# kkty/kmer-sets-compression

Hardware: AMD Instinct MI355X
Metric: Mk-mers/s processed in kmerset-multiple-compress; bytes/k-mer after SPSS (higher is better)
Workload: dtype u32

## Files before the change

kmer-sets-compression_amd/csrc/ksh_encode.hip:

```cpp
#include "ksh_internal.h"
#include "ksh_dsu.h"
#include "ksh_kmer.h"

#include <algorithm>
#include <cstddef>
#include <cstdlib>
#include <string>

namespace ksh {

#ifndef KSH_RULER_SHIFT
#define KSH_RULER_SHIFT 5
#endif
constexpr int kRulerShift = KSH_RULER_SHIFT;
constexpr uint32_t kRulerEvery = 1u << kRulerShift;

constexpr uint32_t kNone = 0xFFFFFFFFu;
constexpr uint32_t kMulti = 0xFFFFFFFEu;

#ifndef KSH_JUMP_HOPS
#define KSH_JUMP_HOPS 4
#endif
constexpr int kJumpHops = KSH_JUMP_HOPS;

#ifdef KSH_TRACE
__device__ unsigned long long* g_probe_trace = nullptr;
__device__ long long g_probe_trace_rows = 0;
#define KSH_PMARK(which, m)                                                                              \
  do {                                                                                                   \
    if (g_probe_trace && threadIdx.x == 0 && int64_t(blockIdx.x) < g_probe_trace_rows)                    \
      g_probe_trace[((which) * g_probe_trace_rows + blockIdx.x) * 16 + (m)] = __builtin_amdgcn_s_memtime(); \
  } while (0)
#define KSH_PMARK_WAVE(which)                                                                            \
  do {                                                                                                   \
    if (g_probe_trace && threadIdx.x % 64 == 0 && threadIdx.x / 64 < 16 && int64_t(blockIdx.x) < g_probe_trace_rows) \
      g_probe_trace[((which) * g_probe_trace_rows + blockIdx.x) * 16 + threadIdx.x / 64] = __builtin_amdgcn_s_memtime(); \
  } while (0)
#else
#define KSH_PMARK(which, m) do { } while (0)
#define KSH_PMARK_WAVE(which) do { } while (0)
// ... 186 lines not shown
                                                      const uint32_t* __restrict__ hist_matrix,
                                                      const int64_t* __restrict__ goff,
                                                      RcRecord<KeyT>* __restrict__ rec) {
  extern __shared__ uint32_t lds_hist[];
  const int nb = 1 << nbits;
  const uint32_t* my_row = hist_matrix + int64_t(blockIdx.x) * nb;
  for (int b = threadIdx.x; b < nb; b += blockDim.x) lds_hist[b] = uint32_t(goff[b]) + my_row[b];
  const int64_t t_begin = int64_t(blockIdx.x) * per_row;
  const int64_t t_end = min(t_begin + per_row, set.n);
  __syncthreads();
  if (t_begin >= t_end) return;
  const int64_t b_first = set.bucket_of(t_begin), b_last = set.bucket_of(t_end - 1);
  const int k = set.k, low_bits = 2 * set.k - 2 - nbits;
  const uint64_t low_mask = (uint64_t(1) << low_bits) - 1;
  for (int64_t t = t_begin + threadIdx.x; t < t_end; t += blockDim.x) {
    const uint64_t key = uint64_t(set.keys[t]);
    const uint32_t grp = uint32_t(revcomp(key, k) >> low_bits) & uint32_t(nb - 1);
    if (int(grp >> (nbits - round_bits)) != round) continue;
    int64_t lo = b_first, hi = b_last;
    while (lo < hi) {
      const int64_t mid = (lo + hi + 1) >> 1;
      if (set.off[mid] <= t) lo = mid; else hi = mid - 1;
    }
    const uint64_t rx = revcomp((uint64_t(lo) << set.key_bits) | key, k);
    const uint32_t dst = atomicAdd(&lds_hist[grp], 1u);
    RcRecord<KeyT> r;
    r.key = KeyT(((rx >> (2 * k - 2)) << low_bits) | (rx & low_mask));
    r.t = uint32_t(t);
    rec[dst] = r;
  }
}

constexpr int kSgBits = 7;
constexpr int kL1Threads = 1024;
constexpr int kL2Threads = 256;
constexpr int kL2Per = 8;
constexpr int kL2Tile = kL2Threads * kL2Per;

template <typename KeyT, int kPer>
__global__ __launch_bounds__(kL1Threads) void k_rc_scatter_l1(DevSet<KeyT> set, int nbits, int64_t per_row,
                                                               const uint32_t* __restrict__ hist_matrix,
                                                               const int64_t* __restrict__ goff,
                                                               RcRecord<KeyT>* __restrict__ tmp_rec,
                                                               uint16_t* __restrict__ tmp_g) {
  constexpr int kTile = kL1Threads * kPer;
  constexpr int kSg = 1 << kSgBits;
  __shared__ RcRecord<KeyT> s_rec[kTile];
  __shared__ uint16_t s_g[kTile];
  __shared__ uint32_t s_cur[kSg], s_cnt[kSg], s_lbase[kSg + 1];
  constexpr int kOffCap = 1024;
  __shared__ int64_t s_off[kOffCap];
  const int tid = threadIdx.x;
  const int nb = 1 << nbits, lo_bits = nbits - kSgBits;
  const uint32_t* my_row = hist_matrix + int64_t(blockIdx.x) * nb;
  if (tid < kSg) {
    uint32_t at = uint32_t(goff[int64_t(tid) << lo_bits]);
    for (int gi = 0; gi < (1 << lo_bits); gi++) at += my_row[(tid << lo_bits) + gi];
    s_cur[tid] = at;
    s_cnt[tid] = 0;
  }
  const int64_t t_begin = int64_t(blockIdx.x) * per_row;
  const int64_t t_end = min(t_begin + per_row, set.n);
  __syncthreads();
  if (t_begin >= t_end) return;
  const int64_t b_first = set.bucket_of(t_begin), b_last = set.bucket_of(t_end - 1);
  const int k = set.k, low_bits = 2 * set.k - 2 - nbits;
  const uint64_t low_mask = (uint64_t(1) << low_bits) - 1;
  const int n_span = int(min<int64_t>(b_last - b_first + 1, kOffCap + 1));
  const bool off_staged = n_span <= kOffCap;
  if (off_staged)
    for (int j = tid; j < n_span; j += kL1Threads) s_off[j] = set.off[b_first + j];
  __syncthreads();
  for (int64_t t0 = t_begin; t0 < t_end; t0 += kTile) {
    const int tile_n = int(min<int64_t>(kTile, t_end - t0));
    RcRecord<KeyT> mine[kPer];
    uint32_t grp[kPer], rank[kPer];
#pragma unroll
    for (int j = 0; j < kPer; j++) {
      const int64_t t = t0 + tid + j * kL1Threads;
      grp[j] = 0xFFFFFFFFu;
      if (t >= t_end) continue;
      const uint64_t key = uint64_t(set.keys[t]);
      int64_t lo = b_first, hi = b_last;
      if (off_staged) {
        int l2 = 0, h2 = n_span - 1;
        while (l2 < h2) {
          const int mid = (l2 + h2 + 1) >> 1;
          if (s_off[mid] <= t) l2 = mid; else h2 = mid - 1;
        }
        lo = b_first + l2;
      } else {
        while (lo < hi) {
          const int64_t mid = (lo + hi + 1) >> 1;
          if (set.off[mid] <= t) lo = mid; else hi = mid - 1;
        }
      }
      const uint64_t rx = revcomp((uint64_t(lo) << set.key_bits) | key, k);
      grp[j] = uint32_t(rx >> low_bits) & uint32_t(nb - 1);
      mine[j].key = KeyT(((rx >> (2 * k - 2)) << low_bits) | (rx & low_mask));
      mine[j].t = uint32_t(t);
      rank[j] = atomicAdd(&s_cnt[grp[j] >> lo_bits], 1u);
    }
    __syncthreads();
    if (tid < 64) {
      static_assert(kSg == 128, "two super-groups per lane of one wave");
      const uint32_t c0 = s_cnt[2 * tid], c1 = s_cnt[2 * tid + 1];
      uint32_t inc = c0 + c1;
#pragma unroll
      for (int d = 1; d < 64; d <<= 1) {
        const uint32_t o = __shfl_up(inc, d, 64);
        if (tid >= d) inc += o;
      }
      s_lbase[2 * tid] = inc - c0 - c1;
      s_lbase[2 * tid + 1] = inc - c1;
    }
    __syncthreads();
#pragma unroll
    for (int j = 0; j < kPer; j++) {
      if (grp[j] == 0xFFFFFFFFu) continue;
      const uint32_t pos = s_lbase[grp[j] >> lo_bits] + rank[j];
      s_rec[pos] = mine[j];
      s_g[pos] = uint16_t(grp[j]);
    }
    __syncthreads();
    for (int i = tid; i < tile_n; i += kL1Threads) {
      const uint32_t sg = uint32_t(s_g[i]) >> lo_bits;
      const uint32_t dst = s_cur[sg] + (uint32_t(i) - s_lbase[sg]);
      tmp_rec[dst] = s_rec[i];
      tmp_g[dst] = s_g[i];
    }
    __syncthreads();
    if (tid < kSg) {
      s_cur[tid] += s_cnt[tid];
      s_cnt[tid] = 0;
    }
    __syncthreads();
  }
}

template <typename KeyT>
__global__ __launch_bounds__(kL2Threads) void k_rc_scatter_l2(int64_t n, int nbits, const int64_t* __restrict__ goff,
                                                               const RcRecord<KeyT>* __restrict__ tmp_rec,
                                                               const uint16_t* __restrict__ tmp_g,
                                                               uint32_t* __restrict__ cursor,
                                                               RcRecord<KeyT>* __restrict__ rec) {
  constexpr int kBins = 512;
  __shared__ RcRecord<KeyT> s_rec[kL2Tile];
  __shared__ uint16_t s_bin[kL2Tile];
  __shared__ uint32_t s_cnt[kBins], s_lbase[kBins], s_gbase[kBins];
  __shared__ uint32_t s_first;
  const int tid = threadIdx.x;
  const int lo_bits = nbits - kSgBits;
  const int64_t p0 = int64_t(blockIdx.x) * kL2Tile;
  const int tile_n = int(min<int64_t>(kL2Tile, n - p0));
  for (int b = tid; b < kBins; b += kL2Threads) s_cnt[b] = 0;
  if (tid == 0) s_first = (uint32_t(tmp_g[p0]) >> lo_bits) << lo_bits;
  __syncthreads();
  const uint32_t base_g = s_first;
  const uint32_t n_bins = min<uint32_t>(uint32_t(kBins), (2u << lo_bits));
  RcRecord<KeyT> mine[kL2Per];
  uint32_t bin[kL2Per], rank[kL2Per];
#pragma unroll
  for (int j = 0; j < kL2Per; j++) {
    const int i = tid + j * kL2Threads;
    bin[j] = 0xFFFFFFFFu;
    if (i >= tile_n) continue;
    mine[j] = tmp_rec[p0 + i];
    const uint32_t g = tmp_g[p0 + i];
    if (g - base_g < n_bins) {
      bin[j] = g - base_g;
      rank[j] = atomicAdd(&s_cnt[bin[j]], 1u);
    } else {
      rec[uint32_t(goff[g]) + atomicAdd(&cursor[g], 1u)] = mine[j];
    }
  }
  __syncthreads();
  {
    static_assert(kBins == 2 * kL2Threads, "two bins per thread");
    __shared__ uint32_t s_wave[kL2Threads / 64];
    const uint32_t c0 = s_cnt[2 * tid], c1 = s_cnt[2 * tid + 1];
    uint32_t inc = c0 + c1;
    const int lane = tid & 63, wv = tid >> 6;
#pragma unroll
    for (int d = 1; d < 64; d <<= 1) {
      const uint32_t o = __shfl_up(inc, d, 64);
      if (lane >= d) inc += o;
    }
    if (lane == 63) s_wave[wv] = inc;
    __syncthreads();
    uint32_t before = inc - (c0 + c1);
    for (int w = 0; w < wv; w++) before += s_wave[w];
    s_lbase[2 * tid] = before;
    s_lbase[2 * tid + 1] = before + c0;
    s_gbase[2 * tid] = c0 ? uint32_t(goff[base_g + 2 * tid]) + atomicAdd(&cursor[base_g + 2 * tid], c0) : 0u;
    s_gbase[2 * tid + 1] = c1 ? uint32_t(goff[base_g + 2 * tid + 1]) + atomicAdd(&cursor[base_g + 2 * tid + 1], c1) : 0u;
  }
  __syncthreads();
#pragma unroll
  for (int j = 0; j < kL2Per; j++) {
    if (bin[j] == 0xFFFFFFFFu) continue;
    const uint32_t pos = s_lbase[bin[j]] + rank[j];
// ... 1124 lines not shown
}

__device__ __forceinline__ unsigned long long rec_look(const unsigned long long* p) {
  return __hip_atomic_load(p, __ATOMIC_RELAXED, __HIP_MEMORY_SCOPE_AGENT);
}
__device__ __forceinline__ void rec_post(unsigned long long* p, unsigned long long v) {
  __hip_atomic_store(p, v, __ATOMIC_RELAXED, __HIP_MEMORY_SCOPE_AGENT);
}
__device__ __forceinline__ bool first_phase(uint32_t s) {
  return (((s >> 1) * 0x9E3779B1u) >> 13 ^ s) & 1u;
}

struct WalkLog {
  unsigned long long* hdr;
  uint32_t* mid;
  int64_t n_walkers;
  int n_mid;
  int k;
  uint32_t* long_walkers;
  unsigned int* long_count;
  uint32_t long_tag;
  __device__ __forceinline__ bool is_long(uint32_t steps) const { return steps > uint32_t(n_mid + 1) * uint32_t(k); }
  __device__ __forceinline__ void arrived(int64_t w, uint32_t steps, uint32_t state) const {
    if (!hdr) return;
    hdr[w] = (uint64_t(steps) << 32) | state;
    if (is_long(steps)) long_walkers[atomicAdd(long_count, 1u)] = uint32_t(w) | long_tag;
  }
  __device__ __forceinline__ void passed(int64_t w, int j, uint32_t state) const {
    if (hdr && j < n_mid) mid[int64_t(j) * n_walkers + w] = state;
  }
};
constexpr int kLogMidRulers = 7, kLogMidHeads = 7;

template <int kPhase>
__global__ __launch_bounds__(256) void k_rank_walk(const uint32_t* __restrict__ link, int64_t n_states,
                                                    int64_t n_dense, unsigned long long* __restrict__ rinfo,
                                                    unsigned long long* __restrict__ chain_info, WalkLog log,
                                                    unsigned long long* __restrict__ unset_a,
                                                    unsigned long long* __restrict__ unset_b) {
  const int64_t i = int64_t(blockIdx.x) * blockDim.x + threadIdx.x;
  if (i >= n_dense) return;
  if (unset_a) {
    unset_a[i] = ~0ull;
    unset_b[i] = ~0ull;
  }
  const int64_t s64 = 2 * int64_t(kRulerEvery) * (i >> 1) + (i & 1);
  if (s64 >= n_states) {
    rinfo[i] = make_rinfo(true, 0, 0);
    return;
  }
  const uint32_t r = uint32_t(s64);
  if (kPhase == 1 && !first_phase(r)) return;
  if (rec_look(rinfo + i) != kRecUnset) return;
  const uint2 own = link_pair(link, r);
  uint32_t lk = leave_link(own, r);
  if (lk == kNone) {
    rec_post(rinfo + i, make_rinfo(true, 0, r));
    if (enter_link(own, r) == kNone) log.arrived(i, 0, r);
    return;
  }
  uint32_t cur = r, steps = 0;
  int since = 0, n_passed = 0;
  while (true) {
    cur = step_to(cur, lk);
    steps++;
    if (sampled_ruler(cur) || steps >= 0x3FFFFFFFu) {
      rec_post(rinfo + i, make_rinfo(false, steps, cur));
      rec_post(rinfo + dense_index(cur ^ 1), make_rinfo(false, steps, r ^ 1));
      log.arrived(i, steps, cur);
      return;
    }
    if (++since == log.k) {
      since = 0;
      log.passed(i, n_passed++, cur);
    }
    lk = leave_link(link_pair(link, cur), cur);
    if (lk == kNone) {
      rec_post(rinfo + i, make_rinfo(true, steps, cur));
      rec_post(chain_info + (cur >> 1), make_chain_info(true, steps, dense_index(r ^ 1)));
      log.arrived(i, steps, cur);
      return;
    }
  }
}

template <int kPhase>
__global__ __launch_bounds__(256) void k_rank_heads(const uint32_t* __restrict__ link,
                                                     const uint32_t* __restrict__ ends, int64_t n_ends,
                                                     unsigned long long* __restrict__ rinfo,
                                                     unsigned long long* __restrict__ chain_info, WalkLog log) {
  const int64_t e = int64_t(blockIdx.x) * blockDim.x + threadIdx.x;
  if (e >= n_ends) return;
  const uint32_t t = ends[e];
  if ((t & (kRulerEvery - 1)) == 0) return;
  const uint2 own = reinterpret_cast<const uint2*>(link)[t];
  uint32_t s0;
  if (own.x == kNone && own.y != kNone) {
    s0 = 2 * t;
  } else if (own.y == kNone && own.x != kNone) {
    s0 = 2 * t + 1;
  } else {
    log.arrived(e, 0, 2 * t);
    return;
  }
  if (kPhase == 1 && !first_phase(s0)) return;
  if (rec_look(chain_info + t) != kRecUnset) return;
  uint32_t lk = leave_link(own, s0);
  uint32_t cur = s0, off = 0;
  int since = 0, n_passed = 0;
  while (true) {
    cur = step_to(cur, lk);
    off++;
    if (sampled_ruler(cur)) {
      rec_post(chain_info + t, make_chain_info(true, off, dense_index(cur)));
      rec_post(rinfo + dense_index(cur ^ 1), make_rinfo(true, off, s0 ^ 1));
      log.arrived(e, off, cur);
      return;
    }
    if (++since == log.k) {
      since = 0;
      log.passed(e, n_passed++, cur);
    }
    lk = leave_link(link_pair(link, cur), cur);
    if (lk == kNone || off >= 0x3FFFFFFFu) {
      rec_post(chain_info + t, make_chain_info(false, off, cur));
      rec_post(chain_info + (cur >> 1), make_chain_info(false, off, s0 ^ 1));
      log.arrived(e, off, cur);
      return;
    }
  }
}

__global__ __launch_bounds__(256) void k_rank_unset(const uint32_t* __restrict__ ends, int64_t n_ends,
                                                     unsigned long long* __restrict__ chain_info) {
  const int64_t e = int64_t(blockIdx.x) * blockDim.x + threadIdx.x;
  if (e < n_ends) chain_info[ends[e]] = kRecUnset;
}

__global__ __launch_bounds__(256) void k_ruler_jump(int64_t n_dense,
                                                     unsigned long long* __restrict__ rinfo,
                                                     const int* __restrict__ prev,
                                                     int* __restrict__ changed) {
  if (prev && *prev == 0) return;
  const int64_t i = int64_t(blockIdx.x) * blockDim.x + threadIdx.x;
  if (i >= n_dense) return;
  uint64_t mine = rinfo[i];
  if (mine & kEndFlag) return;
#pragma unroll
  for (int hop = 0; hop < kJumpHops && !(mine & kEndFlag); hop++) {
    const uint64_t theirs = rinfo[dense_index(uint32_t(mine))];
    const uint32_t dist = uint32_t((mine >> 32) & 0x7FFFFFFFu) + uint32_t((theirs >> 32) & 0x7FFFFFFFu);
    mine = (theirs & kEndFlag) | (uint64_t(dist & 0x7FFFFFFFu) << 32) | uint32_t(theirs);
  }
  rinfo[i] = mine;
  *changed = 1;
}

#ifndef KSH_L2_SHIFT
#define KSH_L2_SHIFT 4
#endif
constexpr int kL2Shift = KSH_L2_SHIFT;
// ... 1193 lines not shown
  uint32_t *u_head = nullptr, *u_first = nullptr, *u_last = nullptr, *u_len = nullptr,
           *edges = nullptr, *mate = nullptr, *best_w = nullptr, *u_sid = nullptr,
           *u_koff = nullptr, *lens = nullptr, *sc_nodes = nullptr, *sc_parent = nullptr,
           *sc_rank = nullptr;
  unsigned long long *best_prio = nullptr, *sc_used = nullptr;
  uint8_t *visited = nullptr, *scls = nullptr, *u_flip = nullptr;
  int64_t *s_nk = nullptr, *sc01 = nullptr, *sc2 = nullptr, *str_start = nullptr;
  EncCtl* ctl = nullptr;
  int rounds = 0;
  int64_t routes = 0;
  bool stamped = true;
  bool directed = false;
  const unsigned long long *rinfo = nullptr, *chain_info = nullptr;
  const uint32_t* ends = nullptr;
  int64_t n_ends = 0;
  WalkLog log_rulers{}, log_heads{};
  bool cover = false;
  ksh_spss_view in{};
  int64_t* in_start = nullptr;
  bool ready = false;
  bool written = false;
  bool ambiguous = false;
};

inline size_t al(size_t x) { return (x + 255) & ~size_t(255); }

#define KSH_BOUND(cond)                                                                              \
  do {                                                                                               \
    if (!(cond)) return ::ksh::fail(KSH_INTERNAL, "encode: bound violated: %s (%s:%d)", #cond, __FILE__, __LINE__); \
  } while (0)
static_assert(sizeof(RcRecord<uint16_t>) == 8 && sizeof(RcRecord<uint32_t>) == 8 && sizeof(RcRecord<uint64_t>) == 16,
              "record sizes the scratch layout assumes");

constexpr int64_t kRcRowsMax = 512;
constexpr int64_t kRcWindowBytes = 78 << 10;

inline bool staged_adjacency() {
  static const bool on = [] {
    const char* e = getenv("KSH_ADJACENCY");
    return !(e && std::string(e) == "probe");
  }();
  return on;
}
inline bool rank_with_stamps() {
  static const bool on = [] {
    const char* e = getenv("KSH_RANK");
    return e && std::string(e) == "stamp";
  }();
  return on;
}
inline bool emit_by_walking() {
  static const bool on = [] {
    const char* e = getenv("KSH_EMIT");
    return e && std::string(e) == "walk";
  }();
  return on;
}
inline int64_t l2_threshold() {
  static const int64_t v = [] {
    const char* e = getenv("KSH_L2_MIN");
    return e ? std::max<int64_t>(4096, atoll(e)) : int64_t(1) << 20;
  }();
  return v;
}
inline unsigned nblk(int64_t n) { return unsigned(std::max<int64_t>(1, (n + 255) / 256)); }

template <typename T>
T* carve(char*& at, size_t count) {
  T* p = reinterpret_cast<T*>(at);
  at += al(count * sizeof(T));
  return p;
}

void free_plan(ksh_ctx* ctx) {
  EncPlan* p = static_cast<EncPlan*>(ctx->enc_state);
  if (!p) return;
  if (p->ublock) pool_free(ctx, p->ublock);
  delete p;
  ctx->enc_state = nullptr;
}

static bool replaces_unwritten(const ksh_ctx* ctx, bool cover) {
  const EncPlan* o = static_cast<const EncPlan*>(ctx->enc_state);
  return o && o->ready && !o->written && o->cover == cover;
}

void retire_plan(ksh_ctx* ctx) {
  if (EncPlan* p = static_cast<EncPlan*>(ctx->enc_state)) p->ready = false;
}

static int enc_fine_bits(const ksh_geom* g, int64_t n) {
  const int64_t nb = n_buckets(g);
  int fine_bits = 0;
  while (fine_bits < 13 && fine_bits + 2 < key_bits(g) && (int64_t(3) << fine_bits) < 2 * (n / nb + 1)) fine_bits++;
  return fine_bits;
}
// ... 176 lines not shown
        const uint32_t bit = 1u << (sizeof(KeyT) == 2 ? 0 : sizeof(KeyT) == 4 ? 1 : 2);
        if (!(ctx->lds_opt_in & bit)) {
          const int bytes = int(kRcWindowBytes + 2048);
          KSH_HIP(hipFuncSetAttribute(reinterpret_cast<const void*>(k_adj_rc<KeyT, 1024>),
                                      hipFuncAttributeMaxDynamicSharedMemorySize, bytes));
          KSH_HIP(hipFuncSetAttribute(reinterpret_cast<const void*>(k_adj_rc<KeyT, 512>),
                                      hipFuncAttributeMaxDynamicSharedMemorySize, bytes));
          KSH_HIP(hipFuncSetAttribute(reinterpret_cast<const void*>(k_adj_rc<KeyT, 256>),
                                      hipFuncAttributeMaxDynamicSharedMemorySize, bytes));
          KSH_HIP(hipFuncSetAttribute(reinterpret_cast<const void*>(k_adj_rc<KeyT, 64>),
                                      hipFuncAttributeMaxDynamicSharedMemorySize, bytes));
          KSH_HIP(hipFuncSetAttribute(reinterpret_cast<const void*>(k_adj_rc1<KeyT, 1024>),
                                      hipFuncAttributeMaxDynamicSharedMemorySize, kRc1LdsBytes));
          KSH_HIP(hipFuncSetAttribute(reinterpret_cast<const void*>(k_adj_rc1<KeyT, 512>),
                                      hipFuncAttributeMaxDynamicSharedMemorySize, kRc1LdsBytes));
          KSH_HIP(hipFuncSetAttribute(reinterpret_cast<const void*>(k_adj_rc1<KeyT, 256>),
                                      hipFuncAttributeMaxDynamicSharedMemorySize, kRc1LdsBytes));
          KSH_HIP(hipFuncSetAttribute(reinterpret_cast<const void*>(k_adj_rc1<KeyT, 64>),
                                      hipFuncAttributeMaxDynamicSharedMemorySize, kRc1LdsBytes));
          KSH_HIP(hipFuncSetAttribute(reinterpret_cast<const void*>(k_rc_hist<KeyT>),
                                      hipFuncAttributeMaxDynamicSharedMemorySize, int(size_t(4) << 15)));
          ctx->lds_opt_in |= bit;
        }
      }
      KSH_BOUND(hist_lds <= (size_t(4) << 15) && ng <= 65536);
      hipLaunchKernelGGL((k_rc_hist<KeyT>), dim3(unsigned(rows)), dim3(1024), hist_lds, st,
                         static_cast<const KeyT*>(sv->d_keys), n, g->k, key_bits(g), gbits, per_row, hist);
      hipLaunchKernelGGL(k_rc_columns, dim3(unsigned((ng + 63) / 64)), dim3(64 * kColTeams), 0, st, hist, rows, int(ng),
                         totals);
      KSH_TRY(scan_exclusive_i64(ctx, totals, goff, ng, goff + ng));
      p->routes |= KSH_ROUTE_PROBE_STAGED | (two_level ? KSH_ROUTE_SCATTER_TWO_LEVEL : 0);
      if (two_level) {
        RcRecord<KeyT>* tmp_rec = sizeof(RcRecord<KeyT>) == 8 ? rec + n : reinterpret_cast<RcRecord<KeyT>*>(p->nbr);
        uint16_t* tmp_g = reinterpret_cast<uint16_t*>(p->head);
        KSH_BOUND(sizeof(RcRecord<KeyT>) == 8 ? size_t(2 * n) * sizeof(RcRecord<KeyT>) <= al(size_t(2 * n) * 8)
                                    : reinterpret_cast<char*>(p->link) == reinterpret_cast<char*>(p->nbr) + al(size_t(2 * n) * 4) &&
                                          size_t(n) * sizeof(RcRecord<KeyT>) <= 2 * al(size_t(2 * n) * 4));
        KSH_BOUND(gbits - kSgBits <= 8);
        uint32_t* cursor = rc_cursor;
        constexpr int kPer = sizeof(RcRecord<KeyT>) == 8 ? 4 : 2;
        hipLaunchKernelGGL((k_rc_scatter_l1<KeyT, kPer>), dim3(unsigned(rows)), dim3(kL1Threads), 0, st, set, gbits,
                           per_row, hist, goff, tmp_rec, tmp_g);
        hipLaunchKernelGGL((k_rc_scatter_l2<KeyT>), dim3(unsigned((n + kL2Tile - 1) / kL2Tile)), dim3(kL2Threads), 0,
                           st, n, gbits, goff, tmp_rec, tmp_g, cursor, rec);
      } else {
        hipLaunchKernelGGL((k_rc_scatter<KeyT>), dim3(unsigned(rows)), dim3(1024), hist_lds, st, set, gbits, 0, 0,
                           per_row, hist, goff, rec);
      }
      const int64_t per_group = n / ng;
      const int cap = int(std::min<int64_t>((kRcWindowBytes - 4 * kRcSegs) / int64_t(sizeof(KeyT) + 6),
                                            std::max<int64_t>(1024, extra ? per_group * 23 / 20 + 256 : per_group * 5 / 4 + 256))) & ~7;
      const size_t rc_lds = size_t(cap) * (sizeof(KeyT) + 4) + size_t(cap + 2 * kRcSegs) * 2;
      KSH_BOUND(cap >= 8 && cap % 8 == 0 && cap + 2 * kRcSegs < 65536);
      KSH_BOUND(rc_lds + 2048 <= size_t(kRcWindowBytes) + 2048 && rc_lds <= size_t(kRcWindowBytes));
      int64_t* pb = static_cast<int64_t*>(arena_alloc(ctx, size_t(ng) * 2 * kRcSegs * 8));
      int64_t* pb0 = extra ? static_cast<int64_t*>(arena_alloc(ctx, size_t(ng) * 2 * 8)) : nullptr;
      if (!pb || (extra && !pb0)) return fail(KSH_INTERNAL, "scratch arena too small");
      hipLaunchKernelGGL((k_rc_bounds<KeyT>), dim3(nblk(ng * 2 * kRcSegs + (extra ? ng * 2 : 0))), dim3(256), 0, st, set,
                         gbits, pb, pb0);
      p->routes |= per_group > 4096 ? KSH_ROUTE_RC_1024 : per_group > 1024 ? KSH_ROUTE_RC_512
                   : per_group > 256 ? KSH_ROUTE_RC_256 : KSH_ROUTE_RC_64;
      static const int rc1_mode = [] {
        const char* e = getenv("KSH_RC1");
        return !e ? 1 : (std::string(e) == "marks" ? 2 : (std::string(e) == "batched" ? 0 : 1));
      }();
      const bool rc1_marks = rc1_mode == 2;
      const int rc1_cap = rc1_marks ? 0 : int(std::min<int64_t>(Rc1Cfg<KeyT>::kCap, (per_group * 4 / 3 + 263) & ~int64_t(7)));
      const int pass1_cap = rc1_marks ? -1 : rc1_cap;
      const bool with_rc = rc1_mode != 0;
      int rc1_sbits = 6;
      while ((1 << rc1_sbits) < kRc1SlicesMax && (2 << rc1_sbits) <= rc1_cap + 1) rc1_sbits++;
      const size_t rc1_lds = (size_t(4) << rc1_sbits) + size_t(rc1_cap) * Rc1Cfg<KeyT>::kEntryBytes;
      KSH_BOUND(rc1_lds <= size_t(kRc1LdsBytes) && rc1_cap % 8 == 0 && rc1_cap < (2 << rc1_sbits) - 1);
      if (!rc1_marks) p->routes |= KSH_ROUTE_RC1_STREAMED;
      const int rc1_batched = rc1_mode == 0 ? 1 : 0;
#define KSH_LAUNCH_RC(T)                                                                                              \
  do {                                                                                                                \
// ... 101 lines not shown
        lr.k = lh.k = g->k;
        const size_t used = (size_t(n_dense) + size_t(n)) * 8;
        const size_t log_bytes = size_t(n_dense) * (8 + 4 * kLogMidRulers + 4) + size_t(n_ends) * (8 + 4 * kLogMidHeads + 4) + 64;
        if (!emit_by_walking() && used + log_bytes <= size_t(2 * n) * 8) {
          unsigned long long* at8 = p->info + n_dense + n;
          lr.hdr = at8;
          lh.hdr = at8 + n_dense;
          uint32_t* at4 = reinterpret_cast<uint32_t*>(at8 + n_dense + n_ends);
          lr.mid = at4;
          lh.mid = at4 + size_t(kLogMidRulers) * n_dense;
          lr.long_walkers = lh.long_walkers = lh.mid + size_t(kLogMidHeads) * n_ends;
          lr.long_count = lh.long_count = ctl->long_count;
          lr.long_tag = 0;
          lh.long_tag = kLongHead;
          lr.n_walkers = n_dense;
          lh.n_walkers = n_ends;
          lr.n_mid = kLogMidRulers;
          lh.n_mid = kLogMidHeads;
          KSH_HIP(hipMemsetAsync(at8, 0xFF, size_t(n_dense + n_ends) * 8, st));
          p->routes |= KSH_ROUTE_EMIT_LOGS;
        }
        p->log_rulers = lr;
        p->log_heads = lh;
        KSH_HIP(hipMemsetAsync(rinfo, 0xFF, size_t(n_dense) * 8, st));
        hipLaunchKernelGGL(k_rank_unset, dim3(nblk(n_ends)), dim3(256), 0, st, ends, n_ends, chain_info);
        static const int64_t race_min = [] {
          const char* e = getenv("KSH_RANK_PHASES");
          if (e && std::string(e) == "1") return int64_t(0);
          if (e && std::string(e) == "2") return int64_t(1) << 60;
          const char* m = getenv("KSH_RANK_RACE_MIN");
          return m ? int64_t(atoll(m)) : int64_t(1) << 18;
        }();
        p->routes |= (n_dense >= race_min ? KSH_ROUTE_RANK_ONE_LAUNCH : 0) | (n_ends >= race_min ? KSH_ROUTE_HEADS_ONE_LAUNCH : 0);
        if (n_dense < race_min)
          hipLaunchKernelGGL(k_rank_walk<1>, dim3(nblk(n_dense)), dim3(256), 0, st, link, ns2, n_dense, rinfo, chain_info, lr,
                             static_cast<unsigned long long*>(nullptr), static_cast<unsigned long long*>(nullptr));
        if (n_ends < race_min)
          hipLaunchKernelGGL(k_rank_heads<1>, dim3(nblk(n_ends)), dim3(256), 0, st, link, ends, n_ends, rinfo, chain_info, lh);
        const bool l2_after = n_dense >= l2_threshold();
        hipLaunchKernelGGL(k_rank_walk<2>, dim3(nblk(n_dense)), dim3(256), 0, st, link, ns2, n_dense, rinfo, chain_info, lr,
                           l2_after ? reinterpret_cast<unsigned long long*>(p->hlen) : nullptr,
                           l2_after ? reinterpret_cast<unsigned long long*>(p->hlast) : nullptr);
        hipLaunchKernelGGL(k_rank_heads<2>, dim3(nblk(n_ends)), dim3(256), 0, st, link, ends, n_ends, rinfo, chain_info, lh);
      }
    }
    const bool two_levels = !stamped && n_dense >= l2_threshold();
    const int64_t n_jump = two_levels ? (((n_dense - 1) >> (kL2Shift + 1)) << 1) + 2 : n_dense;
    unsigned long long* r2 = reinterpret_cast<unsigned long long*>(p->uid);
    unsigned long long* l2_head = reinterpret_cast<unsigned long long*>(p->hlen);
    unsigned long long* l2_stamp = reinterpret_cast<unsigned long long*>(p->hlast);
    if (two_levels) p->routes |= KSH_ROUTE_JUMP_TWO_LEVEL;
    if (stamped) p->routes = (p->routes | KSH_ROUTE_RANK_STAMPED) & ~int64_t(KSH_ROUTE_EMIT_LOGS | KSH_ROUTE_RANK_ONE_LAUNCH | KSH_ROUTE_HEADS_ONE_LAUNCH | KSH_ROUTE_JUMP_TWO_LEVEL);
    if (two_levels) {
      hipLaunchKernelGGL(k_l2_walk<true>, dim3(nblk(n_jump)), dim3(256), 0, st, rinfo, n_dense, r2, l2_head, l2_stamp);
      hipLaunchKernelGGL(k_l2_walk<false>, dim3(nblk(n_dense)), dim3(256), 0, st, rinfo, n_dense, r2, l2_head, l2_stamp);
    }
    int max_rounds = 3;
    for (int64_t x = n_jump; x > 1; x /= (kJumpHops + 1)) max_rounds++;
    max_rounds = std::min(max_rounds, kJumpRoundsMax);
    if (!first_pass) {
      KSH_HIP(hipMemsetAsync(ctl->jump_live, 0, sizeof(ctl->jump_live), st));
      KSH_HIP(hipMemsetAsync(d_tot, 0, (3 + kLenSums) * 8, st));
      KSH_HIP(hipMemsetAsync(ctl->long_count, 0, sizeof(ctl->long_count), st));
    }
    for (int round = 0; round < max_rounds; round++) {
      const int* prev = round ? &ctl->jump_live[round - 1] : nullptr;
      if (two_levels)
        hipLaunchKernelGGL(k_l2_jump, dim3(nblk(n_jump)), dim3(256), 0, st, n_jump, r2, prev, &ctl->jump_live[round]);
      else
        hipLaunchKernelGGL(k_ruler_jump, dim3(nblk(n_dense)), dim3(256), 0, st, n_dense, rinfo, prev,
                           &ctl->jump_live[round]);
    }
    if (two_levels)
      hipLaunchKernelGGL(k_l2_resolve, dim3(nblk(n_dense)), dim3(256), 0, st, n_dense, r2, l2_head, l2_stamp, rinfo);
    int* loop_flag = reinterpret_cast<int*>(d_tot + 2 + kLenSums);
    if (stamped) {
// ... 451 lines not shown
```

Before: 27820.

## Drop tmp_g side array by packing group low bits into record t field

The first scatter level stops writing a separate 16-bit group array. It packs the group's low bits together with a row-relative index into the record's t field and publishes per-row, per-supergroup start offsets. The second level recovers the supergroup and source row by binary searching goff and those shared starts, then rebuilds the global index and group. This removes one global write and one read stream per record, at the cost of extra binary-search work per element and new range constraints on per_row.

```diff
diff --git a/kmer-sets-compression_amd/csrc/ksh_encode.hip b/kmer-sets-compression_amd/csrc/ksh_encode.hip
--- a/kmer-sets-compression_amd/csrc/ksh_encode.hip
+++ b/kmer-sets-compression_amd/csrc/ksh_encode.hip
@@ -258,6 +258,7 @@
 }
 
 constexpr int kSgBits = 7;
+constexpr int64_t kRcRowsMax = 512;
 constexpr int kL1Threads = 1024;
 constexpr int kL2Threads = 256;
 constexpr int kL2Per = 8;
@@ -268,7 +269,7 @@
                                                                const uint32_t* __restrict__ hist_matrix,
                                                                const int64_t* __restrict__ goff,
                                                                RcRecord<KeyT>* __restrict__ tmp_rec,
-                                                               uint16_t* __restrict__ tmp_g) {
+                                                               uint32_t* __restrict__ share) {
   constexpr int kTile = kL1Threads * kPer;
   constexpr int kSg = 1 << kSgBits;
   __shared__ RcRecord<KeyT> s_rec[kTile];
@@ -284,6 +285,7 @@
     for (int gi = 0; gi < (1 << lo_bits); gi++) at += my_row[(tid << lo_bits) + gi];
     s_cur[tid] = at;
     s_cnt[tid] = 0;
+    share[int64_t(tid) * gridDim.x + blockIdx.x] = at;
   }
   const int64_t t_begin = int64_t(blockIdx.x) * per_row;
   const int64_t t_end = min(t_begin + per_row, set.n);
@@ -292,6 +294,7 @@
   const int64_t b_first = set.bucket_of(t_begin), b_last = set.bucket_of(t_end - 1);
   const int k = set.k, low_bits = 2 * set.k - 2 - nbits;
   const uint64_t low_mask = (uint64_t(1) << low_bits) - 1;
+  const uint32_t g_low_mask = (1u << lo_bits) - 1u;
   const int n_span = int(min<int64_t>(b_last - b_first + 1, kOffCap + 1));
   const bool off_staged = n_span <= kOffCap;
   if (off_staged)
@@ -324,7 +327,7 @@
       const uint64_t rx = revcomp((uint64_t(lo) << set.key_bits) | key, k);
       grp[j] = uint32_t(rx >> low_bits) & uint32_t(nb - 1);
       mine[j].key = KeyT(((rx >> (2 * k - 2)) << low_bits) | (rx & low_mask));
-      mine[j].t = uint32_t(t);
+      mine[j].t = (uint32_t(t - t_begin) << lo_bits) | (grp[j] & g_low_mask);
       rank[j] = atomicAdd(&s_cnt[grp[j] >> lo_bits], 1u);
     }
     __syncthreads();
@@ -353,7 +356,6 @@
       const uint32_t sg = uint32_t(s_g[i]) >> lo_bits;
       const uint32_t dst = s_cur[sg] + (uint32_t(i) - s_lbase[sg]);
       tmp_rec[dst] = s_rec[i];
-      tmp_g[dst] = s_g[i];
     }
     __syncthreads();
     if (tid < kSg) {
@@ -364,25 +366,55 @@
   }
 }
 
+template <typename T>
+__device__ __forceinline__ int last_at_most(const T* a, int lo, int hi, uint32_t p, int64_t stride = 1) {
+  while (lo < hi) {
+    const int mid = (lo + hi + 1) >> 1;
+    if (uint32_t(a[mid * stride]) <= p) lo = mid; else hi = mid - 1;
+  }
+  return lo;
+}
+
 template <typename KeyT>
-__global__ __launch_bounds__(kL2Threads) void k_rc_scatter_l2(int64_t n, int nbits, const int64_t* __restrict__ goff,
+__global__ __launch_bounds__(kL2Threads) void k_rc_scatter_l2(int64_t n, int nbits, int64_t per_row, int n_rows,
+                                                               const int64_t* __restrict__ goff,
                                                                const RcRecord<KeyT>* __restrict__ tmp_rec,
-                                                               const uint16_t* __restrict__ tmp_g,
+                                                               const uint32_t* __restrict__ share,
                                                                uint32_t* __restrict__ cursor,
                                                                RcRecord<KeyT>* __restrict__ rec) {
   constexpr int kBins = 512;
+  constexpr int kSg = 1 << kSgBits;
   __shared__ RcRecord<KeyT> s_rec[kL2Tile];
   __shared__ uint16_t s_bin[kL2Tile];
   __shared__ uint32_t s_cnt[kBins], s_lbase[kBins], s_gbase[kBins];
+  static_assert(kBins >= kRcRowsMax, "the share starts borrow s_lbase and s_gbase");
+  uint32_t* const s_share[2] = {s_lbase, s_gbase};
   __shared__ uint32_t s_first;
   const int tid = threadIdx.x;
   const int lo_bits = nbits - kSgBits;
+  const uint32_t g_low_mask = (1u << lo_bits) - 1u;
   const int64_t p0 = int64_t(blockIdx.x) * kL2Tile;
   const int tile_n = int(min<int64_t>(kL2Tile, n - p0));
+  const uint32_t q0 = uint32_t(p0), q_end = q0 + uint32_t(tile_n);
   for (int b = tid; b < kBins; b += kL2Threads) s_cnt[b] = 0;
-  if (tid == 0) s_first = (uint32_t(tmp_g[p0]) >> lo_bits) << lo_bits;
+  if (tid < kSg) {
+    const uint32_t lo = uint32_t(goff[int64_t(tid) << lo_bits]), hi = uint32_t(goff[int64_t(tid + 1) << lo_bits]);
+    if (lo <= q0 && q0 < hi) s_first = uint32_t(tid);
+  }
   __syncthreads();
-  const uint32_t base_g = s_first;
+  const uint32_t sg0 = s_first;
+  const uint32_t base_g = sg0 << lo_bits;
+  const uint32_t end0 = uint32_t(goff[int64_t(sg0 + 1) << lo_bits]);
+  const bool second = q_end > end0;
+  const uint32_t end1 = second ? uint32_t(goff[int64_t(sg0 + 2) << lo_bits]) : end0;
+  for (int r = tid; r < n_rows; r += kL2Threads) {
+    s_share[0][r] = share[int64_t(sg0) * n_rows + r];
+    if (second) s_share[1][r] = share[int64_t(sg0 + 1) * n_rows + r];
+  }
+  __syncthreads();
+  const int row_lo0 = last_at_most(s_share[0], 0, n_rows - 1, q0);
+  const int row_hi0 = last_at_most(s_share[0], row_lo0, n_rows - 1, min(q_end, end0) - 1u);
+  const int row_hi1 = second && end1 > end0 ? last_at_most(s_share[1], 0, n_rows - 1, min(q_end, end1) - 1u) : 0;
   const uint32_t n_bins = min<uint32_t>(uint32_t(kBins), (2u << lo_bits));
   RcRecord<KeyT> mine[kL2Per];
   uint32_t bin[kL2Per], rank[kL2Per];
@@ -392,7 +424,27 @@
     bin[j] = 0xFFFFFFFFu;
     if (i >= tile_n) continue;
     mine[j] = tmp_rec[p0 + i];
-    const uint32_t g = tmp_g[p0 + i];
+  }
+#pragma unroll
+  for (int j = 0; j < kL2Per; j++) {
+    const int i = tid + j * kL2Threads;
+    if (i >= tile_n) continue;
+    const uint32_t q = q0 + uint32_t(i);
+    uint32_t sg;
+    int row;
+    if (q < end0) {
+      sg = sg0;
+      row = last_at_most(s_share[0], row_lo0, row_hi0, q);
+    } else if (q < end1) {
+      sg = sg0 + 1;
+      row = last_at_most(s_share[1], 0, row_hi1, q);
+    } else {
+      sg = uint32_t(last_at_most(goff, int(sg0) + 1, kSg - 1, q, int64_t(1) << lo_bits));
+      row = last_at_most(share + int64_t(sg) * n_rows, 0, n_rows - 1, q);
+    }
+    const uint32_t field = mine[j].t;
+    const uint32_t g = (sg << lo_bits) | (field & g_low_mask);
+    mine[j].t = uint32_t(int64_t(row) * per_row) + (field >> lo_bits);
     if (g - base_g < n_bins) {
       bin[j] = g - base_g;
       rank[j] = atomicAdd(&s_cnt[bin[j]], 1u);
@@ -2937,7 +2989,6 @@
 static_assert(sizeof(RcRecord<uint16_t>) == 8 && sizeof(RcRecord<uint32_t>) == 8 && sizeof(RcRecord<uint64_t>) == 16,
               "record sizes the scratch layout assumes");
 
-constexpr int64_t kRcRowsMax = 512;
 constexpr int64_t kRcWindowBytes = 78 << 10;
 
 inline bool staged_adjacency() {
@@ -3209,7 +3260,9 @@
       p->routes |= KSH_ROUTE_PROBE_STAGED | (two_level ? KSH_ROUTE_SCATTER_TWO_LEVEL : 0);
       if (two_level) {
         RcRecord<KeyT>* tmp_rec = sizeof(RcRecord<KeyT>) == 8 ? rec + n : reinterpret_cast<RcRecord<KeyT>*>(p->nbr);
-        uint16_t* tmp_g = reinterpret_cast<uint16_t*>(p->head);
+        uint32_t* share = p->head;
+        KSH_BOUND((size_t(rows) << kSgBits) * 4 <= al(size_t(n) * 4));
+        KSH_BOUND(per_row <= (int64_t(1) << (32 - (gbits - kSgBits))));
         KSH_BOUND(sizeof(RcRecord<KeyT>) == 8 ? size_t(2 * n) * sizeof(RcRecord<KeyT>) <= al(size_t(2 * n) * 8)
                                     : reinterpret_cast<char*>(p->link) == reinterpret_cast<char*>(p->nbr) + al(size_t(2 * n) * 4) &&
                                           size_t(n) * sizeof(RcRecord<KeyT>) <= 2 * al(size_t(2 * n) * 4));
@@ -3217,9 +3270,9 @@
         uint32_t* cursor = rc_cursor;
         constexpr int kPer = sizeof(RcRecord<KeyT>) == 8 ? 4 : 2;
         hipLaunchKernelGGL((k_rc_scatter_l1<KeyT, kPer>), dim3(unsigned(rows)), dim3(kL1Threads), 0, st, set, gbits,
-                           per_row, hist, goff, tmp_rec, tmp_g);
+                           per_row, hist, goff, tmp_rec, share);
         hipLaunchKernelGGL((k_rc_scatter_l2<KeyT>), dim3(unsigned((n + kL2Tile - 1) / kL2Tile)), dim3(kL2Threads), 0,
-                           st, n, gbits, goff, tmp_rec, tmp_g, cursor, rec);
+                           st, n, gbits, per_row, int(rows), goff, tmp_rec, share, cursor, rec);
       } else {
         hipLaunchKernelGGL((k_rc_scatter<KeyT>), dim3(unsigned(rows)), dim3(1024), hist_lds, st, set, gbits, 0, 0,
                            per_row, hist, goff, rec);
```

After: 27980 (median of 6 runs). Within noise of the previous version (+0.6%).

## Add optional multi-walker-per-thread and nontemporal link loads to rank walks

Applied to the files above, without the earlier changes.

Templates the rank walk and head walk kernels on a walkers-per-thread count and a streaming-load flag. With two walkers, each thread advances two independent chains and issues their link loads together to overlap memory latency; the streaming flag uses nontemporal loads for link pairs. Both default off (MLP=1, NT=0), so the default path behaves like before apart from the restructured code. The multi-walker mode risks divergence and higher register pressure.

```diff
diff --git a/kmer-sets-compression_amd/csrc/ksh_encode.hip b/kmer-sets-compression_amd/csrc/ksh_encode.hip
--- a/kmer-sets-compression_amd/csrc/ksh_encode.hip
+++ b/kmer-sets-compression_amd/csrc/ksh_encode.hip
@@ -6,6 +6,7 @@
 #include <cstddef>
 #include <cstdlib>
 #include <string>
+#include <type_traits>
 
 namespace ksh {
 
@@ -1583,101 +1584,211 @@
 };
 constexpr int kLogMidRulers = 7, kLogMidHeads = 7;
 
-template <int kPhase>
+typedef uint32_t ksh_u32x2 __attribute__((ext_vector_type(2)));
+template <bool kStream>
+__device__ __forceinline__ uint2 walk_link_pair(const uint32_t* __restrict__ link, uint32_t s) {
+  if (!kStream) return link_pair(link, s);
+  const ksh_u32x2 v = __builtin_nontemporal_load(reinterpret_cast<const ksh_u32x2*>(link) + (s >> 1));
+  return make_uint2(v.x, v.y);
+}
+
+template <int kMlp>
+__device__ __forceinline__ bool walkers_live(const bool (&live)[kMlp]) {
+  bool any = false;
+#pragma unroll
+  for (int w = 0; w < kMlp; w++) any |= live[w];
+  return any;
+}
+template <int kMlp, bool kStream>
+__device__ __forceinline__ void walk_read_links(const uint32_t* __restrict__ link, const bool (&live)[kMlp],
+                                                const uint32_t (&cur)[kMlp], uint2 (&pr)[kMlp]) {
+  if (kMlp == 1) {
+    if (live[0]) pr[0] = walk_link_pair<kStream>(link, cur[0]);
+  } else {
+#pragma unroll
+    for (int w = 0; w < kMlp; w++) pr[w] = walk_link_pair<kStream>(link, live[w] ? cur[w] : cur[w ^ 1]);
+  }
+}
+
+#ifndef KSH_RANK_MLP_DEFAULT
+#define KSH_RANK_MLP_DEFAULT 1
+#endif
+#ifndef KSH_LINK_NT_DEFAULT
+#define KSH_LINK_NT_DEFAULT 0
+#endif
+template <int kPhase, int kMlp, bool kStream>
 __global__ __launch_bounds__(256) void k_rank_walk(const uint32_t* __restrict__ link, int64_t n_states,
                                                     int64_t n_dense, unsigned long long* __restrict__ rinfo,
                                                     unsigned long long* __restrict__ chain_info, WalkLog log,
                                                     unsigned long long* __restrict__ unset_a,
                                                     unsigned long long* __restrict__ unset_b) {
-  const int64_t i = int64_t(blockIdx.x) * blockDim.x + threadIdx.x;
-  if (i >= n_dense) return;
-  if (unset_a) {
-    unset_a[i] = ~0ull;
-    unset_b[i] = ~0ull;
-  }
-  const int64_t s64 = 2 * int64_t(kRulerEvery) * (i >> 1) + (i & 1);
-  if (s64 >= n_states) {
-    rinfo[i] = make_rinfo(true, 0, 0);
-    return;
-  }
-  const uint32_t r = uint32_t(s64);
-  if (kPhase == 1 && !first_phase(r)) return;
-  if (rec_look(rinfo + i) != kRecUnset) return;
-  const uint2 own = link_pair(link, r);
-  uint32_t lk = leave_link(own, r);
-  if (lk == kNone) {
-    rec_post(rinfo + i, make_rinfo(true, 0, r));
-    if (enter_link(own, r) == kNone) log.arrived(i, 0, r);
-    return;
-  }
-  uint32_t cur = r, steps = 0;
-  int since = 0, n_passed = 0;
+  const int64_t t = int64_t(blockIdx.x) * blockDim.x + threadIdx.x;
+  const int64_t half = kMlp == 2 ? (n_dense + 1) >> 1 : n_dense;
+  if (t >= half) return;
+  int64_t i[kMlp];
+  uint32_t r[kMlp], cur[kMlp], lk[kMlp], steps[kMlp];
+  int since[kMlp], n_passed[kMlp];
+  bool live[kMlp];
+  unsigned long long look[kMlp];
+  uint2 pr[kMlp];
+#pragma unroll
+  for (int w = 0; w < kMlp; w++) {
+    i[w] = t + w * half;
+    live[w] = i[w] < n_dense;
+    r[w] = 0;
+    if (!live[w]) continue;
+    if (unset_a) {
+      unset_a[i[w]] = ~0ull;
+      unset_b[i[w]] = ~0ull;
+    }
+    const int64_t s64 = 2 * int64_t(kRulerEvery) * (i[w] >> 1) + (i[w] & 1);
+    if (s64 >= n_states) {
+      rinfo[i[w]] = make_rinfo(true, 0, 0);
+      live[w] = false;
+      continue;
+    }
+    r[w] = uint32_t(s64);
+    if (kPhase == 1 && !first_phase(r[w])) live[w] = false;
+  }
+#pragma unroll
+  for (int w = 0; w < kMlp; w++)
+    if (live[w]) look[w] = rec_look(rinfo + i[w]);
+#pragma unroll
+  for (int w = 0; w < kMlp; w++)
+    if (live[w] && look[w] != kRecUnset) live[w] = false;
+#pragma unroll
+  for (int w = 0; w < kMlp; w++)
+    if (live[w]) pr[w] = link_pair(link, r[w]);
+#pragma unroll
+  for (int w = 0; w < kMlp; w++) {
+    cur[w] = r[w];
+    steps[w] = 0;
+    since[w] = n_passed[w] = 0;
+    lk[w] = kNone;
+    if (!live[w]) continue;
+    lk[w] = leave_link(pr[w], r[w]);
+    if (lk[w] == kNone) {
+      rec_post(rinfo + i[w], make_rinfo(true, 0, r[w]));
+      if (enter_link(pr[w], r[w]) == kNone) log.arrived(i[w], 0, r[w]);
+      live[w] = false;
+    }
+  }
+  if (!walkers_live<kMlp>(live)) return;
   while (true) {
-    cur = step_to(cur, lk);
-    steps++;
-    if (sampled_ruler(cur) || steps >= 0x3FFFFFFFu) {
-      rec_post(rinfo + i, make_rinfo(false, steps, cur));
-      rec_post(rinfo + dense_index(cur ^ 1), make_rinfo(false, steps, r ^ 1));
-      log.arrived(i, steps, cur);
-      return;
-    }
-    if (++since == log.k) {
-      since = 0;
-      log.passed(i, n_passed++, cur);
-    }
-    lk = leave_link(link_pair(link, cur), cur);
-    if (lk == kNone) {
-      rec_post(rinfo + i, make_rinfo(true, steps, cur));
-      rec_post(chain_info + (cur >> 1), make_chain_info(true, steps, dense_index(r ^ 1)));
-      log.arrived(i, steps, cur);
-      return;
-    }
-  }
-}
-
-template <int kPhase>
+#pragma unroll
+    for (int w = 0; w < kMlp; w++) {
+      if (!live[w]) continue;
+      cur[w] = step_to(cur[w], lk[w]);
+      steps[w]++;
+      if (sampled_ruler(cur[w]) || steps[w] >= 0x3FFFFFFFu) {
+        rec_post(rinfo + i[w], make_rinfo(false, steps[w], cur[w]));
+        rec_post(rinfo + dense_index(cur[w] ^ 1), make_rinfo(false, steps[w], r[w] ^ 1));
+        log.arrived(i[w], steps[w], cur[w]);
+        live[w] = false;
+        continue;
+      }
+      if (++since[w] == log.k) {
+        since[w] = 0;
+        log.passed(i[w], n_passed[w]++, cur[w]);
+      }
+    }
+    if (!walkers_live<kMlp>(live)) return;
+    walk_read_links<kMlp, kStream>(link, live, cur, pr);
+#pragma unroll
+    for (int w = 0; w < kMlp; w++) {
+      if (!live[w]) continue;
+      lk[w] = leave_link(pr[w], cur[w]);
+      if (lk[w] == kNone) {
+        rec_post(rinfo + i[w], make_rinfo(true, steps[w], cur[w]));
+        rec_post(chain_info + (cur[w] >> 1), make_chain_info(true, steps[w], dense_index(r[w] ^ 1)));
+        log.arrived(i[w], steps[w], cur[w]);
+        live[w] = false;
+      }
+    }
+  }
+}
+
+template <int kPhase, int kMlp, bool kStream>
 __global__ __launch_bounds__(256) void k_rank_heads(const uint32_t* __restrict__ link,
                                                      const uint32_t* __restrict__ ends, int64_t n_ends,
                                                      unsigned long long* __restrict__ rinfo,
                                                      unsigned long long* __restrict__ chain_info, WalkLog log) {
-  const int64_t e = int64_t(blockIdx.x) * blockDim.x + threadIdx.x;
-  if (e >= n_ends) return;
-  const uint32_t t = ends[e];
-  if ((t & (kRulerEvery - 1)) == 0) return;
-  const uint2 own = reinterpret_cast<const uint2*>(link)[t];
-  uint32_t s0;
-  if (own.x == kNone && own.y != kNone) {
-    s0 = 2 * t;
-  } else if (own.y == kNone && own.x != kNone) {
-    s0 = 2 * t + 1;
-  } else {
-    log.arrived(e, 0, 2 * t);
-    return;
-  }
-  if (kPhase == 1 && !first_phase(s0)) return;
-  if (rec_look(chain_info + t) != kRecUnset) return;
-  uint32_t lk = leave_link(own, s0);
-  uint32_t cur = s0, off = 0;
-  int since = 0, n_passed = 0;
+  const int64_t at = int64_t(blockIdx.x) * blockDim.x + threadIdx.x;
+  const int64_t half = kMlp == 2 ? (n_ends + 1) >> 1 : n_ends;
+  if (at >= half) return;
+  int64_t e[kMlp];
+  uint32_t t[kMlp], s0[kMlp], cur[kMlp], lk[kMlp], off[kMlp];
+  int since[kMlp], n_passed[kMlp];
+  bool live[kMlp];
+  unsigned long long look[kMlp];
+  uint2 pr[kMlp];
+#pragma unroll
+  for (int w = 0; w < kMlp; w++) {
+    e[w] = at + w * half;
+    live[w] = e[w] < n_ends;
+    t[w] = live[w] ? ends[e[w]] : 0;
+    if (live[w] && (t[w] & (kRulerEvery - 1)) == 0) live[w] = false;
+  }
+#pragma unroll
+  for (int w = 0; w < kMlp; w++)
+    if (live[w]) pr[w] = reinterpret_cast<const uint2*>(link)[t[w]];
+#pragma unroll
+  for (int w = 0; w < kMlp; w++) {
+    s0[w] = 0;
+    if (!live[w]) continue;
+    if (pr[w].x == kNone && pr[w].y != kNone) {
+      s0[w] = 2 * t[w];
+    } else if (pr[w].y == kNone && pr[w].x != kNone) {
+      s0[w] = 2 * t[w] + 1;
+    } else {
+      log.arrived(e[w], 0, 2 * t[w]);
+      live[w] = false;
+      continue;
+    }
+    if (kPhase == 1 && !first_phase(s0[w])) live[w] = false;
+  }
+#pragma unroll
+  for (int w = 0; w < kMlp; w++)
+    if (live[w]) look[w] = rec_look(chain_info + t[w]);
+#pragma unroll
+  for (int w = 0; w < kMlp; w++) {
+    if (live[w] && look[w] != kRecUnset) live[w] = false;
+    lk[w] = live[w] ? leave_link(pr[w], s0[w]) : kNone;
+    cur[w] = s0[w];
+    off[w] = 0;
+    since[w] = n_passed[w] = 0;
+  }
+  if (!walkers_live<kMlp>(live)) return;
   while (true) {
-    cur = step_to(cur, lk);
-    off++;
-    if (sampled_ruler(cur)) {
-      rec_post(chain_info + t, make_chain_info(true, off, dense_index(cur)));
-      rec_post(rinfo + dense_index(cur ^ 1), make_rinfo(true, off, s0 ^ 1));
-      log.arrived(e, off, cur);
-      return;
-    }
-    if (++since == log.k) {
-      since = 0;
-      log.passed(e, n_passed++, cur);
-    }
-    lk = leave_link(link_pair(link, cur), cur);
-    if (lk == kNone || off >= 0x3FFFFFFFu) {
-      rec_post(chain_info + t, make_chain_info(false, off, cur));
-      rec_post(chain_info + (cur >> 1), make_chain_info(false, off, s0 ^ 1));
-      log.arrived(e, off, cur);
-      return;
+#pragma unroll
+    for (int w = 0; w < kMlp; w++) {
+      if (!live[w]) continue;
+      cur[w] = step_to(cur[w], lk[w]);
+      off[w]++;
+      if (sampled_ruler(cur[w])) {
+        rec_post(chain_info + t[w], make_chain_info(true, off[w], dense_index(cur[w])));
+        rec_post(rinfo + dense_index(cur[w] ^ 1), make_rinfo(true, off[w], s0[w] ^ 1));
+        log.arrived(e[w], off[w], cur[w]);
+        live[w] = false;
+        continue;
+      }
+      if (++since[w] == log.k) {
+        since[w] = 0;
+        log.passed(e[w], n_passed[w]++, cur[w]);
+      }
+    }
+    if (!walkers_live<kMlp>(live)) return;
+    walk_read_links<kMlp, kStream>(link, live, cur, pr);
+#pragma unroll
+    for (int w = 0; w < kMlp; w++) {
+      if (!live[w]) continue;
+      lk[w] = leave_link(pr[w], cur[w]);
+      if (lk[w] == kNone || off[w] >= 0x3FFFFFFFu) {
+        rec_post(chain_info + t[w], make_chain_info(false, off[w], cur[w]));
+        rec_post(chain_info + (cur[w] >> 1), make_chain_info(false, off[w], s0[w] ^ 1));
+        log.arrived(e[w], off[w], cur[w]);
+        live[w] = false;
+      }
     }
   }
 }
@@ -2967,6 +3078,20 @@
     return e ? std::max<int64_t>(4096, atoll(e)) : int64_t(1) << 20;
   }();
   return v;
+}
+inline int rank_mlp() {
+  static const int v = [] {
+    const char* e = getenv("KSH_RANK_MLP");
+    return e ? (std::string(e) == "1" ? 1 : 2) : KSH_RANK_MLP_DEFAULT;
+  }();
+  return v;
+}
+inline bool link_streamed() {
+  static const bool on = [] {
+    const char* e = getenv("KSH_LINK_NT");
+    return e ? std::string(e) == "1" : bool(KSH_LINK_NT_DEFAULT);
+  }();
+  return on;
 }
 inline unsigned nblk(int64_t n) { return unsigned(std::max<int64_t>(1, (n + 255) / 256)); }
 
@@ -3387,16 +3512,31 @@
           return m ? int64_t(atoll(m)) : int64_t(1) << 18;
         }();
         p->routes |= (n_dense >= race_min ? KSH_ROUTE_RANK_ONE_LAUNCH : 0) | (n_ends >= race_min ? KSH_ROUTE_HEADS_ONE_LAUNCH : 0);
-        if (n_dense < race_min)
-          hipLaunchKernelGGL(k_rank_walk<1>, dim3(nblk(n_dense)), dim3(256), 0, st, link, ns2, n_dense, rinfo, chain_info, lr,
-                             static_cast<unsigned long long*>(nullptr), static_cast<unsigned long long*>(nullptr));
-        if (n_ends < race_min)
-          hipLaunchKernelGGL(k_rank_heads<1>, dim3(nblk(n_ends)), dim3(256), 0, st, link, ends, n_ends, rinfo, chain_info, lh);
+        const int mlp = rank_mlp();
+        const auto launch_walk = [&](auto phase, unsigned long long* unset_a, unsigned long long* unset_b) {
+          constexpr int kPhase = decltype(phase)::value;
+          const auto go = [&](auto kernel) {
+            hipLaunchKernelGGL(kernel, dim3(nblk((n_dense + mlp - 1) / mlp)), dim3(256), 0, st, link, ns2, n_dense, rinfo,
+                               chain_info, lr, unset_a, unset_b);
+          };
+          if (link_streamed()) mlp == 2 ? go(k_rank_walk<kPhase, 2, true>) : go(k_rank_walk<kPhase, 1, true>);
+          else mlp == 2 ? go(k_rank_walk<kPhase, 2, false>) : go(k_rank_walk<kPhase, 1, false>);
+        };
+        const auto launch_heads = [&](auto phase) {
+          constexpr int kPhase = decltype(phase)::value;
+          const auto go = [&](auto kernel) {
+            hipLaunchKernelGGL(kernel, dim3(nblk((n_ends + mlp - 1) / mlp)), dim3(256), 0, st, link, ends, n_ends, rinfo,
+                               chain_info, lh);
+          };
+          if (link_streamed()) mlp == 2 ? go(k_rank_heads<kPhase, 2, true>) : go(k_rank_heads<kPhase, 1, true>);
+          else mlp == 2 ? go(k_rank_heads<kPhase, 2, false>) : go(k_rank_heads<kPhase, 1, false>);
+        };
+        if (n_dense < race_min) launch_walk(std::integral_constant<int, 1>{}, nullptr, nullptr);
+        if (n_ends < race_min) launch_heads(std::integral_constant<int, 1>{});
         const bool l2_after = n_dense >= l2_threshold();
-        hipLaunchKernelGGL(k_rank_walk<2>, dim3(nblk(n_dense)), dim3(256), 0, st, link, ns2, n_dense, rinfo, chain_info, lr,
-                           l2_after ? reinterpret_cast<unsigned long long*>(p->hlen) : nullptr,
-                           l2_after ? reinterpret_cast<unsigned long long*>(p->hlast) : nullptr);
-        hipLaunchKernelGGL(k_rank_heads<2>, dim3(nblk(n_ends)), dim3(256), 0, st, link, ends, n_ends, rinfo, chain_info, lh);
+        launch_walk(std::integral_constant<int, 2>{}, l2_after ? reinterpret_cast<unsigned long long*>(p->hlen) : nullptr,
+                    l2_after ? reinterpret_cast<unsigned long long*>(p->hlast) : nullptr);
+        launch_heads(std::integral_constant<int, 2>{});
       }
     }
     const bool two_levels = !stamped && n_dense >= l2_threshold();
```

Result: slower. 27620 before, 26770 after (-3.1%).
